# LimpBunion22/VIT-FPGA

Measured on AMD Instinct MI355X. Metric: images/sec ViT-B/16 224x224, batch 512 per GPU, higher is better.
Workload: dtype bf16; 1 GPU; vit_base 224x224x3 inference, 512 images per GPU resident in HBM, random-init weights (seed 0); global_batch=512, per_gpu_batch=512

## Files before the change

vit-fpga_amd/csrc/kernels_attn.hip:

```cpp
#include <cstdlib>
#include <type_traits>

#include "vh_kernels.h"

namespace vh {

constexpr float kTau = 8.0f;

__device__ __forceinline__ void swap_halves(float v, float& lo_everywhere, float& hi_everywhere) {
    float a = v, b;
    asm volatile("v_mov_b32 %1, %0\n\ts_nop 1\n\tv_permlane32_swap_b32 %0, %1\n\ts_nop 1" : "+v"(a), "=&v"(b));
    lo_everywhere = a;
    hi_everywhere = b;
}
__device__ __forceinline__ float cross_half_max(float v) {
    float a, b;
    swap_halves(v, a, b);
    return fmaxf(a, b);
}
__device__ __forceinline__ float cross_half_sum(float v) {
    float a, b;
    swap_halves(v, a, b);
    return a + b;
}

template <typename T, bool PERSIST, typename TO = T>
__global__ void __launch_bounds__(1024, PERSIST ? 2 : 4)
attention_kernel(const typename T::elem* __restrict__ qkv, typename TO::elem* __restrict__ out,
                 int tokens, int heads, int slabs, int ntiles, int nitems) {
    using elem = typename T::elem;
    using vec8 = typename T::vec8;
    using vec4 = typename T::vec4;
    extern __shared__ __attribute__((aligned(16))) char smem[];
    const int kv_bytes = ntiles * 4096;
    const int buf_bytes = 2 * kv_bytes;

    const int lane = threadIdx.x & 63;
    const int wave = __builtin_amdgcn_readfirstlane(threadIdx.x >> 6);
    const int nw = blockDim.x >> 6;
    const int l31 = lane & 31, hl = lane >> 5;
    const int D = heads * 64;
    const int64_t ld = 3 * (int64_t)D;

    const int lr = lane >> 3, pc = lane & 7;
    const int ngroups = ntiles * 4;
    auto issue_kv = [&](int item, int buf) {
        const int bh = item / slabs;
        const int b = bh / heads, h = bh - b * heads;
        const elem* base = qkv + (int64_t)b * tokens * ld + h * 64;
        char* kdst = smem + buf * buf_bytes;
        for (int g = wave; g < ngroups; g += nw) {
            const int row = g * 8 + lr;
            const int rsrc = row < tokens ? row : tokens - 1;
            const elem* src = base + rsrc * ld;
            const int ck = pc ^ ((row >> 1) & 7);
            const int cv = pc ^ (((row >> 1) & 1) << 2);
            __builtin_amdgcn_global_load_lds((const void __attribute__((address_space(1)))*)(src + D + ck * 8),
                                             (void __attribute__((address_space(3)))*)(kdst + g * 1024), 16, 0, 0);
            __builtin_amdgcn_global_load_lds((const void __attribute__((address_space(1)))*)(src + 2 * D + cv * 8),
                                             (void __attribute__((address_space(3)))*)(kdst + kv_bytes + g * 1024), 16, 0, 0);
        }
    };
    auto load_q = [&](int item, vec8 (&qf)[4]) {
        const int bh = item / slabs, slab = item - bh * slabs;
        const int b = bh / heads, h = bh - b * heads;
        int qrow = (slab * nw + wave) * 32 + l31;
        qrow = qrow < tokens ? qrow : tokens - 1;
        const elem* qp = qkv + ((int64_t)b * tokens + qrow) * ld + h * 64 + 8 * hl;
#pragma unroll
        for (int ks = 0; ks < 4; ++ks) qf[ks] = *(const vec8*)(qp + 16 * ks);
    };

    const int koff = l31 * 128;
    const int kswz = (l31 >> 1) & 7;
    const int g4 = lane >> 4, i16 = lane & 15, tq = i16 >> 2, tp = i16 & 3;
    const int vrow0 = 4 * (g4 >> 1) + tq;
    const int vcolb = (16 * (g4 & 1) + 4 * tp) * 2;

    const int stride = PERSIST ? (int)gridDim.x : nitems;
    int item = blockIdx.x;
    int buf = 0;
    vec8 qf[4], qn[4];
    issue_kv(item, 0);
    load_q(item, qf);

    while (true) {
        const int next = item + stride;
        const bool has_next = PERSIST && next < nitems;
        asm volatile("s_waitcnt vmcnt(0)" ::: "memory");
        __syncthreads();
        if (has_next) {
            issue_kv(next, buf ^ 1);
            load_q(next, qn);
        }

        const int bh = item / slabs, slab = item - bh * slabs;
        const int b = bh / heads, h = bh - b * heads;
        const int q0 = (slab * nw + wave) * 32;
        const char* Ks = smem + buf * buf_bytes;
        const char* Vs = Ks + kv_bytes;

        if (q0 < tokens) {
            f32x16 o0, o1;
#pragma unroll
            for (int r = 0; r < 16; ++r) { o0[r] = 0.f; o1[r] = 0.f; }
            float m2 = -INFINITY;
            float lsum = 0.f;

            const char* kbase = Ks + koff;
            int kofs[4];
#pragma unroll
            for (int ks = 0; ks < 4; ++ks) kofs[ks] = ((2 * ks + hl) ^ kswz) << 4;
            const int vx = ((vrow0 >> 1) & 1) << 6;
            const char* vb0 = Vs + vrow0 * 128 + (vcolb ^ vx);
            const char* vb1 = Vs + vrow0 * 128 + ((vcolb + 64) ^ vx);

            auto qk = [&](int kt) {
                f32x16 s;
#pragma unroll
                for (int r = 0; r < 16; ++r) s[r] = 0.f;
                const char* kp = kbase + kt * 4096;
#pragma unroll
                for (int ks = 0; ks < 4; ++ks) s = T::mfma32(*(const vec8*)(kp + kofs[ks]), qf[ks], s);
                return s;
            };
            struct VFrag { vec8 f[2][2]; };
            auto load_v = [&](int kt) {
                VFrag v;
                const char* v0 = vb0 + kt * 4096;
                const char* v1 = vb1 + kt * 4096;
#pragma unroll
                for (int ks = 0; ks < 2; ++ks) {
                    const vec4 a0 = T::tr_read(v0 + ks * 2048), c0 = T::tr_read(v0 + ks * 2048 + 1024);
                    const vec4 a1 = T::tr_read(v1 + ks * 2048), c1 = T::tr_read(v1 + ks * 2048 + 1024);
#pragma unroll
                    for (int j = 0; j < 4; ++j) { v.f[ks][0][j] = a0[j]; v.f[ks][0][4 + j] = c0[j]; v.f[ks][1][j] = a1[j]; v.f[ks][1][4 + j] = c1[j]; }
                }
                return v;
            };
            auto softmax_pv = [&](int kt, f32x16 s, const VFrag& vfr, auto masked) {
                if constexpr (decltype(masked)::value) {
#pragma unroll
                    for (int r = 0; r < 16; ++r) {
                        const int key = kt * 32 + (r & 3) + 8 * (r >> 2) + 4 * hl;
                        if (key >= tokens) s[r] = -INFINITY;
                    }
                }
                float mx = s[0];
#pragma unroll
                for (int r = 1; r < 16; ++r) mx = fmaxf(mx, s[r]);
                mx = cross_half_max(mx);
                const float mnew = fmaxf(m2, mx);
                if (__builtin_amdgcn_ballot_w64(mnew != m2)) {
                    const float alpha = __builtin_amdgcn_exp2f(m2 - mnew);
                    lsum *= alpha;
#pragma unroll
                    for (int r = 0; r < 16; ++r) { o0[r] *= alpha; o1[r] *= alpha; }
                    m2 = mnew;
                }
                float psum = 0.f;
#pragma unroll
                for (int r = 0; r < 16; ++r) {
                    s[r] = __builtin_amdgcn_exp2f(s[r] - mnew);
                    psum += s[r];
                }
                lsum += psum;
#pragma unroll
                for (int ks = 0; ks < 2; ++ks) {
                    vec8 pf;
#pragma unroll
                    for (int j = 0; j < 8; ++j) pf[j] = (elem)s[8 * ks + j];
                    o0 = T::mfma32(vfr.f[ks][0], pf, o0);
                    o1 = T::mfma32(vfr.f[ks][1], pf, o1);
                }
            };
            f32x16 s_cur = qk(0);
            for (int kt = 0; kt + 1 < ntiles; ++kt) {
                const VFrag vfr = load_v(kt);
                const f32x16 s_nxt = qk(kt + 1);
                softmax_pv(kt, s_cur, vfr, std::false_type{});
                s_cur = s_nxt;
            }
            {
                const VFrag vfr = load_v(ntiles - 1);
                softmax_pv(ntiles - 1, s_cur, vfr, std::true_type{});
            }

            const float ltot = cross_half_sum(lsum);
            const float inv = 1.0f / ltot;
            const int q = q0 + l31;
            if (q < tokens) {
                typename TO::elem* op = out + ((int64_t)b * tokens + q) * D + h * 64 + 4 * hl;
#pragma unroll
                for (int rg = 0; rg < 4; ++rg) {
                    *(typename TO::vec4*)(op + 8 * rg) = pack4<TO>(o0[4 * rg] * inv, o0[4 * rg + 1] * inv, o0[4 * rg + 2] * inv, o0[4 * rg + 3] * inv);
                    *(typename TO::vec4*)(op + 32 + 8 * rg) = pack4<TO>(o1[4 * rg] * inv, o1[4 * rg + 1] * inv, o1[4 * rg + 2] * inv, o1[4 * rg + 3] * inv);
                }
            }
        }
        if (!has_next) break;
        item = next;
        buf ^= 1;
#pragma unroll
        for (int ks = 0; ks < 4; ++ks) qf[ks] = qn[ks];
    }
}

#ifndef VH_ATTN_ABL
#define VH_ATTN_ABL 0
#endif
__device__ __forceinline__ void ring_barrier() {
    __builtin_amdgcn_sched_barrier(0);
    __builtin_amdgcn_s_waitcnt(0xC07F);
    __builtin_amdgcn_s_barrier();
    __builtin_amdgcn_sched_barrier(0);
}
__device__ __forceinline__ void ring_dma16(const void* base, uint32_t lane_off, uint32_t lds_addr) {
    asm_lds_dma16(base, lane_off, lds_addr);
}
#ifdef VH_DIAG_STAMPS
__device__ unsigned long long g_attn_diag[1024 * 16 * 16];
__device__ __forceinline__ unsigned long long attn_rt() {
    unsigned long long t;
    asm volatile("s_memrealtime %0\n\ts_waitcnt lgkmcnt(0)" : "=s"(t)::"memory");
    return t;
}
__device__ __forceinline__ unsigned long long attn_ct() {
    unsigned long long t;
    asm volatile("s_memtime %0\n\ts_waitcnt lgkmcnt(0)" : "=s"(t)::"memory");
    return t;
}
#define VH_ATT_T(i) do { __builtin_amdgcn_sched_barrier(0); const unsigned long long n_ = attn_ct(); ph_[i] += n_ - last_; last_ = n_; __builtin_amdgcn_sched_barrier(0); } while (0)
#else
#define VH_ATT_T(i) do { } while (0)
#endif
__device__ __forceinline__ void ring_wait_vm(int n) {
#define VH_W(N) case N: asm volatile("s_waitcnt vmcnt(" #N ")" ::: "memory"); break;
    switch (n) {
        VH_W(1) VH_W(2) VH_W(3) VH_W(4) VH_W(5) VH_W(6) VH_W(7) VH_W(8) VH_W(9) VH_W(10) VH_W(11) VH_W(12) VH_W(13) VH_W(14)
        VH_W(15) VH_W(16) VH_W(17) VH_W(18) VH_W(19) VH_W(20) VH_W(21) VH_W(22) VH_W(23) VH_W(24) VH_W(25) VH_W(26) VH_W(27)
        VH_W(28) VH_W(29) VH_W(30) VH_W(31) VH_W(32) VH_W(33) VH_W(34) VH_W(35) VH_W(36) VH_W(37) VH_W(38) VH_W(39) VH_W(40)
        default: asm volatile("s_waitcnt vmcnt(0)" ::: "memory"); break;
    }
#undef VH_W
}
__device__ __forceinline__ void ring_wait_dma() {
    asm volatile("s_waitcnt vmcnt(0)" ::: "memory");
}

template <typename T, typename TO = T, bool QS = false, bool OTILE = false, bool IHM = false>
__global__ void __launch_bounds__(1024, 4)
attention_ring_kernel(const typename T::elem* __restrict__ qkv, typename TO::elem* __restrict__ out,
                      int tokens, int heads, int slabs, int ntiles, int nitems, unsigned int* __restrict__ ticket,
                      unsigned int heads_rcp, int64_t hm_rows) {
    using elem = typename T::elem;
    using vec8 = typename T::vec8;
    using vec4 = typename T::vec4;
    extern __shared__ __attribute__((aligned(16))) char smem[];
    const int G = (tokens + 7) >> 3, G2 = (G + 1) & ~1;
    const int kv_bytes = QS ? G * 1024 : ntiles * 4096;
    const int q_off = kv_bytes + (QS ? G2 * 1024 : kv_bytes);
    const uint32_t lds0 = (uint32_t)(uintptr_t)smem;

    const int lane = threadIdx.x & 63;
    const int wave = __builtin_amdgcn_readfirstlane(threadIdx.x >> 6);
    const int nw = blockDim.x >> 6;
    const int l31 = lane & 31, hl = lane >> 5;
    const int D = heads * 64;
    const int64_t ld = IHM ? 64 : 3 * (int64_t)D;
    const uint32_t koff2 = IHM ? (uint32_t)(hm_rows * D * 2) : (uint32_t)(D * 2);
    auto head_base = [&](int b, int h) {
        if constexpr (IHM) return qkv + ((int64_t)h * hm_rows + (int64_t)b * tokens) * 64;
        else return qkv + (int64_t)b * tokens * ld + h * 64;
    };

    auto kv_base = [&](int item) {
        if (QS) {
            const int b = (heads == 1 ? item : (int)__umulhi((unsigned)item, heads_rcp)), h = item - b * heads;
            return head_base(b, h);
        }
        const int bh = item / slabs;
        const int b = bh / heads, h = bh - b * heads;
        return head_base(b, h);
    };
    auto issue_tile = [&](const elem* base, int t) {
        int ln = lane;
        asm volatile("" : "+v"(ln));
        const int lr_ = ln >> 3, pc_ = ln & 7;
        const int g = 4 * t + wave;
        const int gk = QS && g >= G ? G - 1 : g, gv = QS && g >= G2 ? G2 - 1 : g;
        const int rowk = gk * 8 + lr_, rowv = gv * 8 + lr_;
        const int rk = rowk < tokens ? rowk : tokens - 1;
        const int rv = rowv < tokens ? rowv : tokens - 1;
        const int ck = pc_ ^ ((rowk >> 1) & 7);
        const int cv = pc_ ^ (((rowv >> 1) & 1) << 2);
        const uint32_t ok = (uint32_t)(rk * (int)ld + ck * 8) * 2u + koff2;
        const uint32_t ov = (uint32_t)(rv * (int)ld + cv * 8) * 2u + 2u * koff2;
        ring_dma16(base, ok, lds0 + gk * 1024);
        ring_dma16(base, ov, lds0 + kv_bytes + gv * 1024);
    };
    auto issue_q = [&](const elem* base) {
        int ln = lane;
        asm volatile("" : "+v"(ln));
        const int lr_ = ln >> 3, pc_ = ln & 7;
        for (int j = 0; j < nw; ++j) {
            const int g = 4 * j + wave;
            const int row = g * 8 + lr_;
            const int rsrc = row < tokens ? row : tokens - 1;
            const int ck = pc_ ^ ((row >> 1) & 7);
            ring_dma16(base, (uint32_t)(rsrc * (int)ld + ck * 8) * 2u, lds0 + q_off + g * 1024);
        }
    };
    auto load_q = [&](int item, vec8 (&qf)[4]) {
        const int bh = item / slabs, slab = item - bh * slabs;
        const int b = bh / heads, h = bh - b * heads;
        int qrow = (slab * nw + wave) * 32 + l31;
        qrow = qrow < tokens ? qrow : tokens - 1;
        const elem* qp = head_base(b, h) + (int64_t)qrow * ld + 8 * hl;
        asm volatile("global_load_dwordx4 %0, %4, off\n\tglobal_load_dwordx4 %1, %4, off offset:32\n\t"
                     "global_load_dwordx4 %2, %4, off offset:64\n\tglobal_load_dwordx4 %3, %4, off offset:96"
                     : "=&v"(qf[0]), "=&v"(qf[1]), "=&v"(qf[2]), "=&v"(qf[3]) : "v"(qp) : "memory");
    };

    const int kswz = (l31 >> 1) & 7;
    const int g4 = lane >> 4, i16 = lane & 15, tq = i16 >> 2, tp = i16 & 3;
    const int vrow0 = 4 * (g4 >> 1) + tq;
    const int vcolb = (16 * (g4 & 1) + 4 * tp) * 2;
    const int k0 = l31 * 128 + ((hl ^ kswz) << 4);
    const int vx = ((vrow0 >> 1) & 1) << 6;
    const int v0 = kv_bytes + vrow0 * 128 + (vcolb ^ vx);

    const int stride = (int)gridDim.x;
    int item = blockIdx.x * slabs;
    const elem* cbase = kv_base(item);
    vec8 qf[4];
    if (wave < 4) {
        if (QS) issue_q(cbase);
        for (int t = 0; t < ntiles; ++t) issue_tile(cbase, t);
    }
    if (!QS) load_q(item, qf);
    bool first = true;
    constexpr int NST = 4;
    const int w_top = 2 * (ntiles - 2) + NST, w_t1 = 2 * (ntiles - 3) + NST + 2, w_mid = 2 * ntiles + nw - 4 + NST, w_last = nw + 2 + 2 * (ntiles - 3);
    bool stored = false;

#ifdef VH_DIAG_STAMPS
    const unsigned long long rt0_ = attn_rt();
    unsigned int dbg_[3] = {0xffffffffu, 0xffffffffu, 0xffffffffu};
    int dbg_n_ = 0;
    unsigned long long ph_[10] = {0, 0, 0, 0, 0, 0, 0, 0, 0, 0}, last_ = attn_ct();
#endif
    const bool dyn = QS && ticket != nullptr && nw >= 5;
    const int tk_off = q_off + 4 * nw * 1024;
    unsigned int tkv = 0;
    while (true) {
        const int slab_now = QS ? 0 : item - (item / slabs) * slabs;
        const bool last_slab = QS || slab_now + 1 == slabs;
        int next = QS ? item + stride : (last_slab ? (item / slabs + stride) * slabs : item + 1);
        if (QS && dyn && !first) {
            if (wave == nw - 1) {
                if (stored) asm volatile("s_waitcnt vmcnt(%0)" :: "n"(NST) : "memory");
                else asm volatile("s_waitcnt vmcnt(0)" ::: "memory");
                asm volatile("" : "+v"(tkv));
                if (lane == 0) *(volatile unsigned int __attribute__((address_space(3)))*)(uintptr_t)(lds0 + tk_off) = 2u * (unsigned)stride + tkv;
            }
        }
        const int b = QS ? (heads == 1 ? item : (int)__umulhi((unsigned)item, heads_rcp)) : (item / slabs) / heads;
        const int slab = slab_now;
        const int h = (QS ? item : item / slabs) - b * heads;
        const int q0 = (slab * nw + wave) * 32;

        VH_ATT_T(7);
        if (QS) {
            ring_wait_vm(first ? 0 : w_top);
        } else {
            if (first || !stored) asm volatile("s_waitcnt vmcnt(0)" ::: "memory");
            else asm volatile("s_waitcnt vmcnt(%0)" :: "n"(NST) : "memory");
            asm volatile("" : "+v"(qf[0]), "+v"(qf[1]), "+v"(qf[2]), "+v"(qf[3]));
        }
        VH_ATT_T(0);
        ring_barrier();
        VH_ATT_T(1);
        if (QS && dyn && !first) next = __builtin_amdgcn_readfirstlane(*(volatile const int __attribute__((address_space(3)))*)(uintptr_t)(lds0 + tk_off));
#if defined(VH_DIAG_STAMPS) && defined(VH_ATTN_TKDBG)
        if (QS && dyn && !first) { if (dbg_n_ < 3) dbg_[dbg_n_++] = (unsigned)next; next = item + stride; }
#endif
        const bool has_next = (unsigned)next < (unsigned)nitems;
        const bool refill = has_next && last_slab;
        const elem* nbase = kv_base(has_next ? next : item);
        if (QS && dyn && has_next && wave == nw - 1 && lane == 0) {
            asm_atomic_add_ret_issue(ticket, 1u, tkv);
        }
        if (!(VH_ATTN_ABL & 2) && !first && slab == 0 && wave < 4) issue_tile(cbase, ntiles - 1);
        if (QS) {
            int qa = q_off + wave * 4096 + k0;
            if constexpr (!std::is_same<T, TO>::value) {
                int ln = lane;
                asm volatile("" : "+v"(ln));
                const int r31 = ln & 31;
                qa = q_off + wave * 4096 + r31 * 128 + ((((ln >> 5)) ^ ((r31 >> 1) & 7)) << 4);
            }
#pragma unroll
            for (int ks = 0; ks < 4; ++ks) qf[ks] = *(const vec8*)(smem + (qa ^ (ks << 5)));
        }

        f32x16 o0, o1;
#pragma unroll
        for (int r = 0; r < 16; ++r) { o0[r] = 0.f; o1[r] = 0.f; }
        float negm = 0.f;
        float lsum = 0.f;

        auto qk = [&](int kt, float init) {
            int ka = k0 + kt * 4096;
            if constexpr (!std::is_same<T, TO>::value) asm volatile("" : "+v"(ka));
            vec8 kf[4];
#pragma unroll
            for (int ks = 0; ks < 4; ++ks) {
                if (VH_ATTN_ABL & 32) kf[ks] = qf[ks]; else if (VH_ATTN_ABL & 128) kf[ks] = *(const vec8*)(smem + ((ka ^ (ks << 5)) & 0x3ff0)); else
                kf[ks] = *(const vec8*)(smem + (ka ^ (ks << 5)));
            }
            __builtin_amdgcn_sched_barrier(0);
            typedef float f32x2 __attribute__((ext_vector_type(2)));
            typedef float f32x8 __attribute__((ext_vector_type(8)));
            const f32x2 i2 = {init, init};
            f32x2 p[8];
#pragma unroll
            for (int i = 0; i < 8; ++i) asm volatile("v_mov_b64 %0, %1" : "=v"(p[i]) : "v"(i2));
            const f32x4 q0 = __builtin_shufflevector(p[0], p[1], 0, 1, 2, 3), q1 = __builtin_shufflevector(p[2], p[3], 0, 1, 2, 3);
            const f32x4 q2 = __builtin_shufflevector(p[4], p[5], 0, 1, 2, 3), q3 = __builtin_shufflevector(p[6], p[7], 0, 1, 2, 3);
            const f32x8 h0 = __builtin_shufflevector(q0, q1, 0, 1, 2, 3, 4, 5, 6, 7), h1 = __builtin_shufflevector(q2, q3, 0, 1, 2, 3, 4, 5, 6, 7);
            f32x16 s = __builtin_shufflevector(h0, h1, 0, 1, 2, 3, 4, 5, 6, 7, 8, 9, 10, 11, 12, 13, 14, 15);
#pragma unroll
            for (int ks = 0; ks < 4; ++ks) {
                if (VH_ATTN_ABL & 16) s[ks] += (float)kf[ks][0] * (float)qf[ks][0];
                else s = T::mfma32(kf[ks], qf[ks], s);
            }
            return s;
        };
        struct VFrag { vec8 f[2][2]; };
        auto load_v = [&](int kt) {
            VFrag v;
            if (VH_ATTN_ABL & 32) { for (int ks = 0; ks < 2; ++ks) { v.f[ks][0] = qf[ks]; v.f[ks][1] = qf[ks + 2]; } return v; }
            const char* p0 = smem + (v0 + kt * 4096);
            const char* p1 = smem + ((v0 + kt * 4096) ^ 64);
#pragma unroll
            for (int ks = 0; ks < 2; ++ks) {
                const vec4 a0 = T::tr_read(p0 + ks * 2048), c0 = T::tr_read(p0 + ks * 2048 + 1024);
                const vec4 a1 = T::tr_read(p1 + ks * 2048), c1 = T::tr_read(p1 + ks * 2048 + 1024);
#pragma unroll
                for (int j = 0; j < 4; ++j) { v.f[ks][0][j] = a0[j]; v.f[ks][0][4 + j] = c0[j]; v.f[ks][1][j] = a1[j]; v.f[ks][1][4 + j] = c1[j]; }
            }
            return v;
        };
        auto softmax_pv = [&](int kt, f32x16& s, const VFrag& vfr, auto first_c, auto tail_c) {
            constexpr bool FIRST = decltype(first_c)::value, TAIL = decltype(tail_c)::value;
            int ng = 4;
            if constexpr (TAIL) {
                const int valid = tokens - kt * 32;
                ng = (valid + 7) >> 3;
#pragma unroll
                for (int g = 0; g < 4; ++g)
                    if (g < ng) {
#pragma unroll
                        for (int j = 0; j < 4; ++j)
                            if (8 * g + j + 4 * hl >= valid) s[4 * g + j] = -INFINITY;
                    }
            }
            float mx = -INFINITY;
#pragma unroll
            for (int g = 0; g < 4; ++g)
                if (!TAIL || g < ng) {
#pragma unroll
                    for (int j = 0; j < 4; ++j) mx = fmaxf(mx, s[4 * g + j]);
                }
            if (VH_ATTN_ABL & 64) mx = s[kt & 15];
            else
            mx = cross_half_max(mx);
            if constexpr (FIRST) {
                negm = -mx;
#pragma unroll
                for (int r = 0; r < 16; ++r) s[r] -= mx;
            } else if (__builtin_amdgcn_ballot_w64(mx > kTau)) {
                const float delta = fmaxf(mx, 0.f);
                const float alpha = __builtin_amdgcn_exp2f(-delta);
                negm -= delta;
                lsum *= alpha;
#pragma unroll
                for (int r = 0; r < 16; ++r) { o0[r] *= alpha; o1[r] *= alpha; s[r] -= delta; }
            }
            typedef float f32x2 __attribute__((ext_vector_type(2)));
            f32x2 psum = {0.f, 0.f};
#pragma unroll
            for (int g = 0; g < 4; ++g) {
                if (!TAIL || g < ng) {
#pragma unroll
                    for (int j = 0; j < 4; ++j) s[4 * g + j] = (VH_ATTN_ABL & 1) ? s[4 * g + j] * 0.001f + 1.0f : __builtin_amdgcn_exp2f(s[4 * g + j]);
                    psum += f32x2{s[4 * g], s[4 * g + 1]};
                    psum += f32x2{s[4 * g + 2], s[4 * g + 3]};
                } else {
#pragma unroll
                    for (int j = 0; j < 4; ++j) s[4 * g + j] = 0.f;
                }
            }
            lsum += psum[0] + psum[1];
#pragma unroll
            for (int ks = 0; ks < 2; ++ks) {
                if (!TAIL || 2 * ks < ng) {
                    vec8 pf;
#pragma unroll
                    for (int j = 0; j < 8; ++j) pf[j] = (elem)s[8 * ks + j];
                    if (VH_ATTN_ABL & 8) { o0[ks] += (float)pf[0]; o1[ks] += (float)vfr.f[ks][0][0] + (float)vfr.f[ks][1][0]; }
                    else {
                    o0 = T::mfma32(vfr.f[ks][0], pf, o0);
                    o1 = T::mfma32(vfr.f[ks][1], pf, o1);
                    }
                }
            }
        };

        {
            const VFrag vfr = load_v(0);
            f32x16 sc = qk(0, 0.f);
            softmax_pv(0, sc, vfr, std::true_type{}, std::false_type{});
        }
        VH_ATT_T(2);
        for (int kt = 1; kt + 1 < ntiles; ++kt) {
            if (QS) ring_wait_vm(kt == 1 ? w_t1 : !has_next ? 0 : w_mid);
            VH_ATT_T(4);
            if (!(VH_ATTN_ABL & 4)) ring_barrier();
            VH_ATT_T(3);
            if (QS && kt == 1 && has_next && wave < 4) issue_q(nbase);
            if (!(VH_ATTN_ABL & 2) && refill && wave < 4) issue_tile(nbase, kt - 1);
            const VFrag vfr = load_v(kt);
            f32x16 sc = qk(kt, negm);
            softmax_pv(kt, sc, vfr, std::false_type{}, std::false_type{});
        }
        VH_ATT_T(4);
        if (QS) ring_wait_vm(!has_next ? 0 : w_last);
        else ring_wait_dma();
        VH_ATT_T(5);
        if (!(VH_ATTN_ABL & 4)) ring_barrier();
        VH_ATT_T(6);
        if (!(VH_ATTN_ABL & 2) && refill && wave < 4) issue_tile(nbase, ntiles - 2);
        {
            const VFrag vfr = load_v(ntiles - 1);
            f32x16 sc = qk(ntiles - 1, negm);
            if (!QS && has_next) load_q(next, qf);
            softmax_pv(ntiles - 1, sc, vfr, std::false_type{}, std::true_type{});
            VH_ATT_T(8);

            const float ltot = cross_half_sum(lsum);
            const float inv = __builtin_amdgcn_rcpf(ltot);
            const int q = q0 + l31;
            if constexpr (sizeof(typename TO::elem) == 2) {
                const int64_t mrow = (int64_t)b * tokens + (q < tokens ? q : tokens - 1);
                typename TO::elem* const op = OTILE ? out + ((mrow >> 4) * (D >> 3) + h * 8 + hl) * 128 + (mrow & 15) * 8
                                                    : out + mrow * D + h * 64 + 8 * hl;
                constexpr int CH = OTILE ? 128 : 8;
#pragma unroll
                for (int db = 0; db < 2; ++db) {
                    const f32x16& o = db ? o1 : o0;
#pragma unroll
                    for (int rg = 0; rg < 4; rg += 2) {
                        const u32x2 ga = __builtin_bit_cast(u32x2, pack4<TO>(o[4 * rg] * inv, o[4 * rg + 1] * inv, o[4 * rg + 2] * inv, o[4 * rg + 3] * inv));
                        const u32x2 gb = __builtin_bit_cast(u32x2, pack4<TO>(o[4 * rg + 4] * inv, o[4 * rg + 5] * inv, o[4 * rg + 6] * inv, o[4 * rg + 7] * inv));
                        const auto sx = __builtin_amdgcn_permlane32_swap(ga[0], gb[0], false, false);
                        const auto sy = __builtin_amdgcn_permlane32_swap(ga[1], gb[1], false, false);
                        if (q < tokens) *(u32x4*)(op + (4 * db + rg) * CH) = u32x4{sx[0], sy[0], sx[1], sy[1]};
                    }
                }
            } else {
                const int64_t mrow = (int64_t)b * tokens + (q < tokens ? q : tokens - 1);
                typename TO::elem* const op = OTILE ? out + ((mrow >> 4) * (D >> 4) + h * 4) * 256 + (mrow & 15) * 16 + 8 * hl
                                                    : out + mrow * D + h * 64 + 8 * hl;
#pragma unroll
                for (int db = 0; db < 2; ++db) {
                    const f32x16& o = db ? o1 : o0;
#pragma unroll
                    for (int rg = 0; rg < 4; rg += 2) {
                        const uint32_t ga = pack4<TO>(o[4 * rg] * inv, o[4 * rg + 1] * inv, o[4 * rg + 2] * inv, o[4 * rg + 3] * inv);
                        const uint32_t gb = pack4<TO>(o[4 * rg + 4] * inv, o[4 * rg + 5] * inv, o[4 * rg + 6] * inv, o[4 * rg + 7] * inv);
                        const auto sx = __builtin_amdgcn_permlane32_swap(ga, gb, false, false);
                        if (q < tokens) *(u32x2*)(op + (OTILE ? (2 * db + (rg >> 1)) * 256 : 32 * db + 8 * rg)) = u32x2{sx[0], sx[1]};
                    }
                }
            }
        }
        VH_ATT_T(9);
        if (!has_next) break;
        stored = q0 < tokens;
        item = next;
        cbase = nbase;
        first = false;
    }
#ifdef VH_DIAG_STAMPS
    VH_ATT_T(7);
    if (lane == 0 && blockIdx.x < 1024) {
#pragma unroll
        for (int i = 0; i < 10; ++i) g_attn_diag[((size_t)blockIdx.x * 16 + wave) * 16 + i] = ph_[i];
        unsigned int hw;
        asm volatile("s_getreg_b32 %0, hwreg(HW_REG_HW_ID)" : "=s"(hw));
        unsigned int xcc;
        asm volatile("s_getreg_b32 %0, hwreg(HW_REG_XCC_ID)" : "=s"(xcc));
        g_attn_diag[((size_t)blockIdx.x * 16 + wave) * 16 + 10] = rt0_;
        g_attn_diag[((size_t)blockIdx.x * 16 + wave) * 16 + 11] = attn_rt();
        g_attn_diag[((size_t)blockIdx.x * 16 + wave) * 16 + 12] = ((unsigned long long)xcc << 32) | hw;
        for (int i = 0; i < 3; ++i) g_attn_diag[((size_t)blockIdx.x * 16 + wave) * 16 + 13 + i] = dbg_[i];
    }
#endif
}

#ifdef VH_DIAG_STAMPS
extern "C" int vh_diag_attn_read(unsigned long long* host, int n_words) {
    return (int)hipMemcpyFromSymbol(host, HIP_SYMBOL(g_attn_diag), (size_t)n_words * 8);
}
#endif

size_t attention_lds_bytes(int tokens) { return (size_t)((tokens + 31) / 32) * 8192; }

static int attn_form(int batch, int tokens, int heads) {
    const int ntiles = (tokens + 31) / 32, nqb = ntiles;
    static const int max_waves = [] { const int e = env_int("VH_ATTN_WAVES", 16); return e < 1 || e > 16 ? 16 : e; }();
    const int slabs = (nqb + max_waves - 1) / max_waves, nw = (nqb + slabs - 1) / slabs;
    static const int want_ring = env_int("VH_ATTN_RING", 1);
    const int G = (tokens + 7) / 8, G2 = (G + 1) & ~1;
    const size_t qs_lds = (size_t)(G + G2 + 4 * nw) * 1024 + 16;
    if (attention_lds_bytes(tokens) > 160 * 1024) return -1;
    if (want_ring >= 1 && want_ring != 2 && slabs == 1 && nw >= 4 && 2 * qs_lds <= 160 * 1024) return 2;
    if (want_ring && ntiles >= 3 && nw >= 4) return 1;
    (void)batch; (void)heads;
    return 0;
}
bool attention_tiled_applies(int batch, int tokens, int heads) { return attn_form(batch, tokens, heads) >= 1 && heads % 2 == 0; }

template <typename T, typename TO = T, bool OTILE = false, bool IHM = false>
static hipError_t launch_attn_t(const void* qkv, int batch, int tokens, int heads, void* out, unsigned int* ticket, hipStream_t s, bool tk_zeroed,
                                int64_t hm_rows = 0) {
    const int ntiles = (tokens + 31) / 32;
    const int nqb = ntiles;
    static const int max_waves = [] { const int e = env_int("VH_ATTN_WAVES", 16); return e < 1 || e > 16 ? 16 : e; }();
    const int slabs = (nqb + max_waves - 1) / max_waves;
    const int nw = (nqb + slabs - 1) / slabs;
    const size_t one = attention_lds_bytes(tokens);
    if (one > 160 * 1024) return hipErrorInvalidValue;
    const int nitems = batch * heads * slabs;
    const int num_cu = device_num_cu();
    if (!num_cu) return hipErrorUnknown;
    static const int want_persist = env_int("VH_ATTN_PERSIST", 0);
    const bool persist = want_persist && 2 * one <= 160 * 1024 && nitems > num_cu;
    static const int want_ring = env_int("VH_ATTN_RING", 1);
    const int G = (tokens + 7) / 8, G2 = (G + 1) & ~1;
    const size_t qs_lds = (size_t)(G + G2 + 4 * nw) * 1024 + 16;
    if (want_ring >= 1 && want_ring != 2 && slabs == 1 && nw >= 4 && 2 * qs_lds <= 160 * 1024) {
        auto k = attention_ring_kernel<T, TO, true, OTILE, IHM>;
        static LdsDone lds_done;
        if (hipError_t e = ensure_dynamic_lds((const void*)k, qs_lds, lds_done); e != hipSuccess) return e;
        const int grid = nitems < 2 * num_cu ? nitems : 2 * num_cu;
        static const int want_dyn = env_int("VH_ATTN_DYN", 1);
        unsigned int* tk = want_dyn && nw >= 5 && nitems > 2 * grid ? ticket : nullptr;
        if (tk && !tk_zeroed) { if (hipError_t e = hipMemsetAsync(tk, 0, sizeof(unsigned int), s); e != hipSuccess) return e; }
        const unsigned int heads_rcp = (unsigned int)(((1ull << 32) + (unsigned)heads - 1) / (unsigned)heads);
        hipLaunchKernelGGL(k, dim3(grid), dim3(nw * 64), qs_lds, s, (const typename T::elem*)qkv, (typename TO::elem*)out,
                           tokens, heads, slabs, ntiles, nitems, tk, heads_rcp, hm_rows);
        return hipGetLastError();
    }
    if (want_ring && ntiles >= 3 && nw >= 4) {
        auto k = attention_ring_kernel<T, TO, false, OTILE, IHM>;
        static LdsDone lds_done;
        if (hipError_t e = ensure_dynamic_lds((const void*)k, one, lds_done); e != hipSuccess) return e;
        const int per_cu = (int)(160 * 1024 / one);
        int grid = num_cu * (per_cu < 1 ? 1 : (per_cu > 2 ? 2 : per_cu));
        if (grid > batch * heads) grid = batch * heads;
        hipLaunchKernelGGL(k, dim3(grid), dim3(nw * 64), one, s, (const typename T::elem*)qkv, (typename TO::elem*)out,
                           tokens, heads, slabs, ntiles, nitems, (unsigned int*)nullptr, 0u, hm_rows);
        return hipGetLastError();
    }
    if constexpr (OTILE) return hipErrorInvalidValue;
    else
    if constexpr (!std::is_same<T, TO>::value) {
        auto k = attention_kernel<T, false, TO>;
        static LdsDone lds_done;
        if (hipError_t e = ensure_dynamic_lds((const void*)k, one, lds_done); e != hipSuccess) return e;
        hipLaunchKernelGGL(k, dim3(nitems), dim3(nw * 64), one, s, (const typename T::elem*)qkv, (typename TO::elem*)out,
                           tokens, heads, slabs, ntiles, nitems);
        return hipGetLastError();
    } else
    if (persist) {
        const size_t lds = 2 * one;
        auto k = attention_kernel<T, true>;
        static LdsDone lds_done;
        if (hipError_t e = ensure_dynamic_lds((const void*)k, lds, lds_done); e != hipSuccess) return e;
        const int per_cu = (int)(160 * 1024 / lds);
        int grid = num_cu * (per_cu < 1 ? 1 : per_cu);
        if (grid > nitems) grid = nitems;
        hipLaunchKernelGGL(k, dim3(grid), dim3(nw * 64), lds, s, (const typename T::elem*)qkv, (typename T::elem*)out,
                           tokens, heads, slabs, ntiles, nitems);
    } else {
        auto k = attention_kernel<T, false>;
        static LdsDone lds_done;
        if (hipError_t e = ensure_dynamic_lds((const void*)k, one, lds_done); e != hipSuccess) return e;
        hipLaunchKernelGGL(k, dim3(nitems), dim3(nw * 64), one, s, (const typename T::elem*)qkv, (typename T::elem*)out,
                           tokens, heads, slabs, ntiles, nitems);
    }
    return hipGetLastError();
}

template <typename T>
__global__ void __launch_bounds__(256)
attention_cls_kernel(const typename T::elem* __restrict__ qkv, typename T::elem* __restrict__ out, int batch, int tokens, int heads) {
    using elem = typename T::elem;
    using vec8 = typename T::vec8;
    constexpr int MAXT = 1024;
    __shared__ float sc[4][MAXT];
    const int lane = threadIdx.x & 63, wv = threadIdx.x >> 6;
    const int item = blockIdx.x * 4 + wv;
    if (item >= batch * heads) return;
    const int b = item / heads, h = item - b * heads;
    const int D = heads * 64;
    const int64_t ld = 3 * (int64_t)D;
    const elem* const base = qkv + (int64_t)b * tokens * ld + h * 64;
    const int g = lane >> 3, c = lane & 7;
    float q[8];
    {
        const vec8 v = *(const vec8*)(base + c * 8);
#pragma unroll
        for (int j = 0; j < 8; ++j) q[j] = (float)v[j];
    }
    float mx = -INFINITY;
    constexpr int U = 4;
    for (int t0 = 0; t0 < tokens; t0 += 8 * U) {
        vec8 v[U];
#pragma unroll
        for (int u = 0; u < U; ++u) {
            const int t = t0 + 8 * u + g;
            v[u] = *(const vec8*)(base + (t < tokens ? t : tokens - 1) * ld + D + c * 8);
        }
#pragma unroll
        for (int u = 0; u < U; ++u) {
            const int t = t0 + 8 * u + g;
            float sv = 0.f;
#pragma unroll
            for (int j = 0; j < 8; ++j) sv = fmaf(q[j], (float)v[u][j], sv);
            sv += __shfl_xor(sv, 1); sv += __shfl_xor(sv, 2); sv += __shfl_xor(sv, 4);
            if (t < tokens) {
                if (c == 0) sc[wv][t] = sv;
                mx = fmaxf(mx, sv);
            }
        }
    }
#pragma unroll
    for (int o = 32; o > 0; o >>= 1) mx = fmaxf(mx, __shfl_xor(mx, o));
    __builtin_amdgcn_s_waitcnt(0xC07F);
    float sum = 0.f;
    for (int t = lane; t < tokens; t += 64) {
        const float p = __builtin_amdgcn_exp2f(sc[wv][t] - mx);
        sc[wv][t] = p;
        sum += p;
    }
#pragma unroll
    for (int o = 32; o > 0; o >>= 1) sum += __shfl_xor(sum, o);
    __builtin_amdgcn_s_waitcnt(0xC07F);
    float acc[8] = {0.f, 0.f, 0.f, 0.f, 0.f, 0.f, 0.f, 0.f};
    for (int t0 = 0; t0 < tokens; t0 += 8 * U) {
        vec8 v[U];
#pragma unroll
        for (int u = 0; u < U; ++u) {
            const int t = t0 + 8 * u + g;
            v[u] = *(const vec8*)(base + (t < tokens ? t : tokens - 1) * ld + 2 * D + c * 8);
        }
#pragma unroll
        for (int u = 0; u < U; ++u) {
            const int t = t0 + 8 * u + g;
            const float p = t < tokens ? sc[wv][t] : 0.f;
#pragma unroll
            for (int j = 0; j < 8; ++j) acc[j] = fmaf(p, (float)v[u][j], acc[j]);
        }
    }
#pragma unroll
    for (int j = 0; j < 8; ++j) {
        acc[j] += __shfl_xor(acc[j], 8); acc[j] += __shfl_xor(acc[j], 16); acc[j] += __shfl_xor(acc[j], 32);
    }
    if (g == 0) {
        const float r = 1.0f / sum;
        vec8 o;
#pragma unroll
        for (int j = 0; j < 8; ++j) o[j] = (elem)(acc[j] * r);
        *(vec8*)(out + (int64_t)b * D + h * 64 + c * 8) = o;
    }
}
hipError_t launch_attention_cls(const void* qkv16, int batch, int tokens, int heads, void* out16, int dtype, hipStream_t s) {
    if (batch <= 0 || tokens <= 0 || tokens > 1024 || heads <= 0) return hipErrorInvalidValue;
    const dim3 grid((unsigned)((batch * heads + 3) / 4));
    if (dtype == VH_DTYPE_BF16)
        hipLaunchKernelGGL(attention_cls_kernel<BF16>, grid, dim3(256), 0, s, (const BF16::elem*)qkv16, (BF16::elem*)out16, batch, tokens, heads);
    else if (dtype == VH_DTYPE_FP16)
        hipLaunchKernelGGL(attention_cls_kernel<FP16>, grid, dim3(256), 0, s, (const FP16::elem*)qkv16, (FP16::elem*)out16, batch, tokens, heads);
    else
        return hipErrorInvalidValue;
    return hipGetLastError();
}

hipError_t launch_attention(const void* qkv16, int batch, int tokens, int heads, void* out16, int dtype,
                            unsigned int* ticket, hipStream_t s, bool ticket_zeroed, bool out_tiled, int64_t in_hm_rows) {
    if (batch <= 0 || tokens <= 0 || heads <= 0) return hipErrorInvalidValue;
    if (in_hm_rows) {
        if (!out_tiled || in_hm_rows < (int64_t)batch * tokens || in_hm_rows * heads * 64 * 4 >= (1ll << 32)) return hipErrorInvalidValue;
        if (!attention_tiled_applies(batch, tokens, heads)) return hipErrorInvalidValue;
        if (dtype == VH_DTYPE_FP8) return launch_attn_t<BF16, E4M3, true, true>(qkv16, batch, tokens, heads, out16, ticket, s, ticket_zeroed, in_hm_rows);
        return dtype == VH_DTYPE_BF16 ? launch_attn_t<BF16, BF16, true, true>(qkv16, batch, tokens, heads, out16, ticket, s, ticket_zeroed, in_hm_rows)
                                      : launch_attn_t<FP16, FP16, true, true>(qkv16, batch, tokens, heads, out16, ticket, s, ticket_zeroed, in_hm_rows);
    }
    if (out_tiled) {
        if (!attention_tiled_applies(batch, tokens, heads)) return hipErrorInvalidValue;
        if (dtype == VH_DTYPE_FP8) return launch_attn_t<BF16, E4M3, true>(qkv16, batch, tokens, heads, out16, ticket, s, ticket_zeroed);
        return dtype == VH_DTYPE_BF16 ? launch_attn_t<BF16, BF16, true>(qkv16, batch, tokens, heads, out16, ticket, s, ticket_zeroed)
                                      : launch_attn_t<FP16, FP16, true>(qkv16, batch, tokens, heads, out16, ticket, s, ticket_zeroed);
    }
    if (attention_lds_bytes(tokens) > 160 * 1024) return launch_attention_stream(qkv16, batch, tokens, heads, out16, dtype, s);
    if (dtype == VH_DTYPE_FP8) return launch_attn_t<BF16, E4M3>(qkv16, batch, tokens, heads, out16, ticket, s, ticket_zeroed);
    return dtype == VH_DTYPE_BF16 ? launch_attn_t<BF16>(qkv16, batch, tokens, heads, out16, ticket, s, ticket_zeroed)
                                  : launch_attn_t<FP16>(qkv16, batch, tokens, heads, out16, ticket, s, ticket_zeroed);
}

}
```

Measured before the change: 28760 images/s.

## Prefetch next K tile from LDS during QK MFMAs and add iglp scheduling

Splits the K-fragment LDS read out of the QK step so the next tile's K fragments are read right after the current tile's MFMAs are issued, overlapping LDS latency with compute. The ring wait counts are adjusted for the earlier reads, and the wait before the last tile moves into the loop. It also inserts an iglp_opt scheduling hint before the PV MFMAs. This raises register pressure (K fragments live across iterations) and reshuffles the ring synchronisation, which risks occupancy loss or wrong-wait hazards.

```diff
diff --git a/vit-fpga_amd/csrc/kernels_attn.hip b/vit-fpga_amd/csrc/kernels_attn.hip
--- a/vit-fpga_amd/csrc/kernels_attn.hip
+++ b/vit-fpga_amd/csrc/kernels_attn.hip
@@ -208,6 +208,9 @@
 
 #ifndef VH_ATTN_ABL
 #define VH_ATTN_ABL 0
+#endif
+#ifndef VH_ATTN_SCHED
+#define VH_ATTN_SCHED 3
 #endif
 __device__ __forceinline__ void ring_barrier() {
     __builtin_amdgcn_sched_barrier(0);
@@ -341,7 +344,10 @@
     if (!QS) load_q(item, qf);
     bool first = true;
     constexpr int NST = 4;
-    const int w_top = 2 * (ntiles - 2) + NST, w_t1 = 2 * (ntiles - 3) + NST + 2, w_mid = 2 * ntiles + nw - 4 + NST, w_last = nw + 2 + 2 * (ntiles - 3);
+    constexpr bool KPF = (VH_ATTN_SCHED & 1) != 0 && std::is_same<T, TO>::value && (QS || OTILE);
+    constexpr int PFS = QS && KPF ? 2 : 0;
+    const int w_top = 2 * (ntiles - 2) + NST - PFS, w_t1 = 2 * (ntiles - 3) + NST + 2 - PFS, w_mid = 2 * ntiles + nw - 4 + NST - PFS,
+              w_last = nw + 2 + 2 * (ntiles - 3) - PFS;
     bool stored = false;
 
 #ifdef VH_DIAG_STAMPS
@@ -410,15 +416,18 @@
         float negm = 0.f;
         float lsum = 0.f;
 
-        auto qk = [&](int kt, float init) {
+        vec8 kf[4];
+        auto read_k = [&](int kt) {
             int ka = k0 + kt * 4096;
             if constexpr (!std::is_same<T, TO>::value) asm volatile("" : "+v"(ka));
-            vec8 kf[4];
 #pragma unroll
             for (int ks = 0; ks < 4; ++ks) {
                 if (VH_ATTN_ABL & 32) kf[ks] = qf[ks]; else if (VH_ATTN_ABL & 128) kf[ks] = *(const vec8*)(smem + ((ka ^ (ks << 5)) & 0x3ff0)); else
                 kf[ks] = *(const vec8*)(smem + (ka ^ (ks << 5)));
             }
+        };
+        auto qk = [&](int kt, float init, int pf_kt) {
+            if (!KPF || pf_kt == -2) read_k(kt);
             __builtin_amdgcn_sched_barrier(0);
             typedef float f32x2 __attribute__((ext_vector_type(2)));
             typedef float f32x8 __attribute__((ext_vector_type(8)));
@@ -434,6 +443,11 @@
             for (int ks = 0; ks < 4; ++ks) {
                 if (VH_ATTN_ABL & 16) s[ks] += (float)kf[ks][0] * (float)qf[ks][0];
                 else s = T::mfma32(kf[ks], qf[ks], s);
+            }
+            if (KPF && pf_kt >= 0) {
+                __builtin_amdgcn_sched_barrier(0);
+                read_k(pf_kt);
+                __builtin_amdgcn_sched_barrier(0);
             }
             return s;
         };
@@ -503,6 +517,7 @@
                 }
             }
             lsum += psum[0] + psum[1];
+            if constexpr ((VH_ATTN_SCHED & 2) != 0) __builtin_amdgcn_iglp_opt(0);
 #pragma unroll
             for (int ks = 0; ks < 2; ++ks) {
                 if (!TAIL || 2 * ks < ng) {
@@ -520,23 +535,26 @@
 
         {
             const VFrag vfr = load_v(0);
-            f32x16 sc = qk(0, 0.f);
+            if (KPF) read_k(0);
+            f32x16 sc = qk(0, 0.f, 1);
             softmax_pv(0, sc, vfr, std::true_type{}, std::false_type{});
         }
         VH_ATT_T(2);
         for (int kt = 1; kt + 1 < ntiles; ++kt) {
-            if (QS) ring_wait_vm(kt == 1 ? w_t1 : !has_next ? 0 : w_mid);
+            if (QS && !KPF) ring_wait_vm(kt == 1 ? w_t1 : !has_next ? 0 : w_mid);
+            else if (QS) ring_wait_vm(kt + 2 == ntiles ? (has_next && kt > 1 ? w_last : 0) : kt == 1 ? w_t1 : !has_next ? 0 : w_mid);
             VH_ATT_T(4);
             if (!(VH_ATTN_ABL & 4)) ring_barrier();
             VH_ATT_T(3);
             if (QS && kt == 1 && has_next && wave < 4) issue_q(nbase);
             if (!(VH_ATTN_ABL & 2) && refill && wave < 4) issue_tile(nbase, kt - 1);
             const VFrag vfr = load_v(kt);
-            f32x16 sc = qk(kt, negm);
+            f32x16 sc = qk(kt, negm, QS || kt + 2 < ntiles ? kt + 1 : -1);
             softmax_pv(kt, sc, vfr, std::false_type{}, std::false_type{});
         }
         VH_ATT_T(4);
-        if (QS) ring_wait_vm(!has_next ? 0 : w_last);
+        if (QS && !KPF) ring_wait_vm(!has_next ? 0 : w_last);
+        else if (QS) { }
         else ring_wait_dma();
         VH_ATT_T(5);
         if (!(VH_ATTN_ABL & 4)) ring_barrier();
@@ -544,7 +562,7 @@
         if (!(VH_ATTN_ABL & 2) && refill && wave < 4) issue_tile(nbase, ntiles - 2);
         {
             const VFrag vfr = load_v(ntiles - 1);
-            f32x16 sc = qk(ntiles - 1, negm);
+            f32x16 sc = qk(ntiles - 1, negm, QS ? -1 : -2);
             if (!QS && has_next) load_q(next, qf);
             softmax_pv(ntiles - 1, sc, vfr, std::false_type{}, std::true_type{});
             VH_ATT_T(8);
```

Measured after the change: 28780 images/s (median of 2 runs). Within noise of the previous version (+0.1%).
